# jaeyoungchoilab/Topsicle

Measured on AMD Instinct MI355X. Metric: bases_scanned_per_sec, higher is better.
Workload: dtype u8

## Files before the change

topsicle_amd/csrc/tps_device.h:

```cpp
#pragma once
#include <stdint.h>
#include "../../include/topsicle_hip.h"

#ifdef TPS_EMU
#define TPS_DEV static inline
#define TPS_HD static inline
#define TPS_PHASE for (int tid = 0; tid < tps::NT; ++tid)
#define TPS_SYNC() ((void)0)
#define TPS_UNROLL
#define TPS_NOVEC
#define TPS_PIN_S(x) ((void)0)
#define TPS_PIN_V(x) ((void)0)
#else
#define TPS_DEV __device__ __forceinline__
#define TPS_HD __host__ __device__ inline
__device__ __forceinline__ int tps_fresh_lane() {
    int t = (int)(threadIdx.x & 63u);
    asm volatile("" : "+v"(t));
    return t;
}
#define TPS_PHASE for (int tid = tps_fresh_lane(), once_ = 1; once_; once_ = 0)
#define TPS_SYNC() do { __builtin_amdgcn_fence(__ATOMIC_SEQ_CST, "wavefront"); __builtin_amdgcn_wave_barrier(); } while (0)
#define TPS_UNROLL _Pragma("unroll")
#define TPS_NOVEC _Pragma("clang loop vectorize(disable) interleave(disable) unroll(disable)")
// ... 89 lines not shown
TPS_DEV uint32_t lut_at(const uint32_t* lut, uint32_t v4, uint32_t amask) { return *(const uint32_t*)((const char*)lut + (v4 & amask)); }
#define lut_at_tile lut_at
#else
TPS_DEV uint32_t lut_at(const uint32_t* lut, uint32_t v4, uint32_t amask) {
    typedef const __attribute__((address_space(3))) uint32_t* lptr_t;
    const uint32_t base = (uint32_t)(uintptr_t)(lptr_t)lut;
    return *(lptr_t)(uintptr_t)((v4 & amask) | base);
}
#ifdef TPS_DIAG_NOCONF
TPS_DEV uint32_t lut_at_tile(const uint32_t* lut, uint32_t v4, uint32_t amask) {
    typedef const __attribute__((address_space(3))) uint32_t* lptr_t;
    const uint32_t base = (uint32_t)(uintptr_t)(lptr_t)lut;
    return *(lptr_t)(uintptr_t)((((v4 & amask) >> 30) | ((threadIdx.x & 63u) << 2)) | base);
}
#else
#define lut_at_tile lut_at
#endif
#endif

#ifndef TPS_WIDE16_MODE
#define TPS_WIDE16_MODE 1
#endif
#ifdef TPS_EMU
TPS_DEV uint32_t lut16_at(const uint32_t* lut, uint32_t v2, uint32_t amask1) { return *(const uint16_t*)((const char*)lut + (v2 & amask1)); }
#define lut16_at_wide lut16_at
#else
TPS_DEV uint32_t lut16_at(const uint32_t* lut, uint32_t v2, uint32_t amask1) {
    typedef const __attribute__((address_space(3))) uint16_t* lptr16_t;
    const uint32_t base = (uint32_t)(uintptr_t)(const __attribute__((address_space(3))) uint32_t*)lut;
    return *(lptr16_t)(uintptr_t)((v2 & amask1) | base);
}
TPS_DEV uint32_t lut16_at_wide(const uint32_t* lut, uint32_t v2, uint32_t amask1) {
    uint32_t h = lut16_at(lut, v2, amask1);
#if TPS_WIDE16_MODE == 1
    asm("" : "+v"(h));
#endif
    return h;
}
#endif

#ifdef TPS_EMU
TPS_DEV void g16_store(uint64_t base, uint32_t i, uint32_t v) { ((uint16_t*)(uintptr_t)base)[i] = (uint16_t)v; }
TPS_DEV uint32_t g16_load(uint64_t base, uint32_t i) { return ((const uint16_t*)(uintptr_t)base)[i]; }
#else
TPS_DEV void g16_store(uint64_t base, uint32_t i, uint32_t v) {
    typedef __attribute__((address_space(1))) uint16_t* gp_t;
    ((gp_t)(uintptr_t)base)[i] = (uint16_t)v;
}
TPS_DEV uint32_t g16_load(uint64_t base, uint32_t i) {
    typedef const __attribute__((address_space(1))) uint16_t* gp_t;
    return ((gp_t)(uintptr_t)base)[i];
}
#endif

#ifdef TPS_EMU
TPS_DEV void g32_store(uint64_t base, uint32_t i, uint32_t v) { ((uint32_t*)(uintptr_t)base)[i] = v; }
TPS_DEV uint32_t g32_load(uint64_t base, uint32_t i) { return ((const uint32_t*)(uintptr_t)base)[i]; }
#else
TPS_DEV void g32_store(uint64_t base, uint32_t i, uint32_t v) {
    typedef __attribute__((address_space(1))) uint32_t* gp_t;
    ((gp_t)(uintptr_t)base)[i] = v;
}
TPS_DEV uint32_t g32_load(uint64_t base, uint32_t i) {
    typedef const __attribute__((address_space(1))) uint32_t* gp_t;
    return ((gp_t)(uintptr_t)base)[i];
}
#endif

TPS_DEV uint32_t mulhi32(uint32_t x, uint32_t y) { return (uint32_t)(((uint64_t)x * (uint64_t)y) >> 32); }
#ifdef TPS_EMU
TPS_DEV uint32_t mul24(uint32_t x, uint32_t y) { return (x & 0xFFFFFFu) * (y & 0xFFFFFFu); }
#else
TPS_DEV uint32_t mul24(uint32_t x, uint32_t y) { return (x & 0xFFFFFFu) * (y & 0xFFFFFFu); }
#endif
#ifdef TPS_EMU
TPS_DEV uint32_t add_bytes(uint32_t v, uint32_t acc) { return acc + (v & 255u) + ((v >> 8) & 255u) + ((v >> 16) & 255u) + (v >> 24); }
#else
TPS_DEV uint32_t add_bytes(uint32_t v, uint32_t acc) { return __builtin_amdgcn_sad_u8(v, 0u, acc); }
#endif

constexpr int cgcd(int a, int b) { return b == 0 ? a : cgcd(b, a % b); }
constexpr int clog2(int x) { return x <= 1 ? 0 : 1 + clog2(x / 2); }

#if defined(TPS_EMU) || !defined(TPS_STAMPS)
#define TPS_STAMP(i) ((void)0)
#else
#define TPS_STAMP(i) do { if (a.stamps && (threadIdx.x & 63u) == 0) a.stamps[r * 16 + (i)] = __builtin_readcyclecounter(); } while (0)
#endif
#if defined(TPS_EMU) || !defined(TPS_STAMPS)
#define TPS_PP_STAMP(i) ((void)0)
#else
#define TPS_PP_STAMP(i) do { if (w0 == 0 && a.stamps && (threadIdx.x & 63u) == 0) a.stamps[tc.rd * 16 + (i)] = __builtin_readcyclecounter(); } while (0)
#endif

struct PatInfo {
    int32_t P, k;
    uint32_t kmask;
    uint32_t all_mask;
    uint32_t so_mask;
    uint32_t dup_mask;
    int32_t n_periods;
    int32_t period[8];
    uint32_t period_pat[8];
    uint32_t hash_mul, hash_shift;
};

struct ScanArgs {
    const uint32_t* seq2;
    const uint16_t* inv;
    const tps_read_desc* desc;
    const uint8_t* tails_in;
    const uint32_t* lut;
    const uint32_t* lut_img;
    const uint32_t* pair_img;
    tps_read_result* results;
    int32_t* c_start;
    int32_t* c_end;
    const int64_t* win_off;
    int32_t* sums;
    uint16_t* sums16;
    const int64_t* win_off16;
    uint8_t* raw;
    uint64_t* stamps;
    int32_t raw_m;
    const int64_t* raw_win_off;
    const int32_t* order;
    int64_t n_reads;
    PatInfo pat;
    tps_params prm;
    int32_t variant;
    int32_t lut_n;
    int32_t seq_dw;
    int32_t head_dw;
    int32_t nblk_cap;
    int32_t spans_per_tile;
    int32_t span_dw;
    int32_t blk_log2;
    int32_t rec_rs;
    int32_t tot_dw;
    int32_t blk_dw;
    int32_t lc_cap;
    uint32_t jump_magic;
    int32_t q, r, lw;
    int32_t lc16;
    int32_t lc_global;
    int32_t lc_stride;
    uint16_t* lc_scratch;
    int32_t pair_n;
    int32_t tile_cap;
    int32_t tw;
    uint32_t tw_magic;
    int32_t tile_full;
    int32_t wpg;
    int32_t pp_d;
    int32_t so_fast;
    int32_t val_on;
    int32_t seq_alias;
    int32_t lut_fields;
    int32_t lut16;
    int32_t xt_alias;
    int32_t xt_own;
    int32_t pair16;
};

struct BinsegArgs {
    const int32_t* sums;
    const int64_t* win_off;
    int32_t* bkp;
    double* gain;
    int64_t n_reads;
// ... 774 lines not shown
    uint64_t lc_g;
    uint16_t* sw16;
    int64_t rd;
};
TPS_DEV TileConst tile_const(const ScanArgs& a, int64_t r) {
    TileConst t;
    t.lc_g = a.lc_global ? (uint64_t)(uintptr_t)(a.lc_scratch + r * (int64_t)a.lc_stride) : 0ull;
    t.sw16 = a.sums16 + (a.win_off16 ? a.win_off16[r] : 0);
    t.rd = r;
    t.q = (int32_t)uniform((uint32_t)a.q); t.r = (int32_t)uniform((uint32_t)a.r);
    t.jump = uniform((uint32_t)a.prm.jump); t.jump_magic = uniform(a.jump_magic);
    t.lc_cap = uniform((uint32_t)a.lc_cap); t.lc16 = uniform((uint32_t)a.lc16);
    TPS_PIN_S(t.q); TPS_PIN_S(t.r); TPS_PIN_S(t.jump); TPS_PIN_S(t.jump_magic); TPS_PIN_S(t.lc_cap); TPS_PIN_S(t.lc16);
    return t;
}

#ifndef TPS_RAW_M
#define TPS_RAW_M 1
#endif
template <int S>
struct Geo {
    static constexpr int B = 8;
    static constexpr int LOG2B = 3;
    static constexpr int C = 8;
    static constexpr int LOG2C = 3;
    static constexpr int POS = B * S;
    static constexpr int WDW = (POS + 13 + 15) / 16;
};
constexpr int SEQ_LEAD = 4;
template <int S, bool FULL>
struct TileGeo {
    static constexpr int LANES = FULL ? NT : NT - 1;
    static constexpr int BASES = LANES * Geo<S>::POS + 13 + 15;
    static constexpr int NQ = (63 + BASES + 63) / 64;
    static constexpr int PF = (NQ + NT - 1) / NT;
    static constexpr int SEQ_TILE = SEQ_LEAD + 4 * NQ + 4;
    static constexpr int SEQ = SEQ_TILE < 144 ? 144 : SEQ_TILE;
};
constexpr bool tile_full_default(int s) { return s >= 1; }

template <int S, bool FULL, int XM = 0>
TPS_DEV Lds carve_fused(uint32_t* base, uint32_t* lut, const ScanArgs& a) {
    constexpr bool XTA = XM == 1;
    constexpr int BLK = 9 * NT + (XM == 0 ? 2 : XM == 1 ? 1 : 0) * XLANES, ROW = NT * Geo<S>::B + NT, SEQ = TileGeo<S, FULL>::SEQ;
    const int VAL = a.val_on ? ((SEQ + 4 + 3) / 4) * 2 : 0;
    static_assert(BLK % 4 == 0 && ROW % 4 == 0 && MISC_DW % 4 == 0 && SEQ % 4 == 0, "seq2 must be 16-byte aligned");
    static_assert(BLK + ROW - SEQ >= HIST_DW && BLK + ROW - SEQ >= 4 * NT, "step 1 counts in front of the aliased bases");
    Lds l;
    l.lut2 = lut - a.pair_n;
    l.lut = lut;
    l.lshift = (a.lut16 && !a.lut_fields && !a.pair16) ? LUT_M16 : (a.lut_fields && a.lut16) ? LUT_F16 : a.lut_fields ? LUT_FIELDS : 16;
    l.blk = base;
    l.XPC = base;
    l.XF = base + 9 * NT;
    l.XT = l.XF + XLANES;
    l.G = l.Gp = base; l.C0 = l.C1 = (uint16_t*)base;
    l.row = base + BLK;
    l.misc = l.row + ROW;
    l.Tot = l.misc + MISC_DW;
    uint32_t* p = l.Tot + 4;
    if (a.seq_alias) {
        l.seq2 = base + (BLK + ROW - SEQ);
    } else {
        l.seq2 = p;
        p += SEQ;
    }
    l.val = (uint16_t*)p;
    p += VAL;
    l.Lc = p;
    l.Lc16 = (uint16_t*)p;
    l.Tc = p + ((a.lc16 && a.lc_global) ? 0 : ((a.lc_cap + 3) / 4) * 2);
    if (XTA) l.XT = a.xt_own ? p + lc_dw(a) : l.seq2;
    if (XM == 2) {
        l.XF = p + lc_dw(a);
        l.XT = l.XF + XLANES;
    }
    return l;
}

#ifdef TPS_EMU
inline int& emu_counter(int i) { static int c[8] = {0, 0, 0, 0, 0, 0, 0, 0}; return c[i]; }
#endif
TPS_DEV uint32_t pack_hi_lo(uint32_t hi_src, uint32_t lo_src) { return perm(hi_src, lo_src, 0x07060100u); }

template <int S, bool SO, bool INV, int RPT, bool PAIR, bool RAW>
TPS_DEV void tile_fused_s(const ScanArgs& a, const TileConst& tc, const Lds& l, int delta, int w0, int tile, int nw_tile,
                          int64_t out_base, uint64_t& s_total, int64_t r) {
    constexpr bool RZ = RPT == 0;
    typedef Geo<S> g_;
    constexpr int WDW = g_::WDW, B = g_::B, LOG2B = g_::LOG2B, POS = g_::POS;
    constexpr int RS = NT + NT / B;
    const PatInfo& pat = a.pat;
    const int rp = RPT >= 0 ? RPT : tc.r, q = tc.q;
    const uint32_t amask = pat.kmask << 2;
    TPS_PHASE {
        const int span = tid;
        const int p0 = delta + span * POS;
        const uint32_t sh2 = (uint32_t)((p0 - 1) & 15) * 2u;
        const int d0 = (p0 - 1) >> 4;
        uint32_t w[WDW];
        {
            uint32_t prev = l.seq2[d0];
            TPS_UNROLL
            for (int i = 0; i < WDW; ++i) {
                uint32_t nx = l.seq2[d0 + i + 1];
                w[i] = alignbit(nx, prev, sh2);
                prev = nx;
            }
        }
        uint32_t cnt = 0, run_or = 0;
        uint32_t gs[B], c0s[B];
        uint32_t* xs = l.row + span * (B + 1);
        uint32_t* xpc = l.XPC + span * (B + 1);
        if constexpr (PAIR) {
            static_assert(!SO && !INV, "pair lookups need per-position independence");
            constexpr int NP = S / 2, NH = NP + (S & 1);
            const uint32_t amask2 = (pat.kmask << 4) | 0xCu;
            const int rpe = rp & ~1;
            uint32_t hc[NH], hn[NH];
            auto v4_at = [&](int p) -> uint32_t {
                const int dw = p >> 4, bit = p & 15;
                return bit ? alignbit(dw + 1 < WDW ? w[dw + 1] : 0u, w[dw], 2u * bit) : w[dw];
            };
            auto fetch = [&](int blk, uint32_t* hh) {
                TPS_UNROLL
                for (int j = 0; j < NP; ++j) hh[j] = lut_at(l.lut2, v4_at(blk * S + 2 * j), amask2);
                if (S & 1) hh[NP] = lut_at(l.lut, v4_at(blk * S + S - 1), amask);
            };
            fetch(0, hc);
            TPS_UNROLL
            for (int blk = 0; blk < B; ++blk) {
                if (blk + 1 < B) fetch(blk + 1, hn);
                uint32_t g = 0;
                c0s[blk] = cnt;
                if (RZ) xpc[blk] = pack_hi_lo(run_or, cnt);
                TPS_UNROLL
                for (int j = 0; j < NH; ++j) {
                    if (!RZ) {
                        if (2 * j == rpe) {
                            uint32_t c1 = cnt, pp = run_or | g;
                            if (rp & 1) {
                                const uint32_t h1 = lut_at(l.lut, v4_at(blk * S + 2 * j), amask);
                                c1 += h1;
                                pp |= h1;
                            }
                            xpc[blk] = pack_hi_lo(pp, c1);
                        }
                    }
                    g |= hc[j];
                    cnt += hc[j];
                }
                gs[blk] = g;
                run_or |= g;
                TPS_UNROLL
                for (int j = 0; j < NH; ++j) hc[j] = hn[j];
            }
        } else {
            uint32_t hc[S], hn[S];
            auto fetch = [&](int blk, uint32_t* hh, int cnt_) {
                TPS_UNROLL
                for (int i = 0; i < S; ++i) {
                    if (i < cnt_) {
                        const int p = blk * S + i;
                        const int dw = p >> 4, bit = p & 15;
                        uint32_t v4 = bit ? alignbit(dw + 1 < WDW ? w[dw + 1] : 0u, w[dw], 2u * bit) : w[dw];
                        uint32_t h;
// ... 269 lines not shown
        TPS_PHASE {
            const uint32_t carry = (uint32_t)s_total;
            if (tid == 0) { l.misc[M_INVALID] = 0; l.misc[M_NTIE] = 0; }
            if (tc.lc16 && tid == 0) l.Tc[tile] = carry;
            uint32_t c = c_lo + (uint32_t)tid;
            uint32_t w = c * jump - (uint32_t)w0;
            TPS_NOVEC
            for (int t = 0; t < passes; ++t) {
                if (c < c_hi) {
                    const uint32_t pre = l.row[w + (w >> LOG2B)];
                    if (tc.lc16) {
                        if (tc.lc_g) g16_store(tc.lc_g, c, pre);
                        else l.Lc16[c] = (uint16_t)pre;
                    } else if (tc.lc_g) {
                        g32_store(tc.lc_g, c, carry + pre);
                    } else {
                        l.Lc[c] = carry + pre;
                    }
                }
                c += NT;
                w += NT * jump;
            }
        }
    }
    s_total += gsum;
    TPS_SYNC();
}

TPS_DEV void tile_candidates(const TileConst& tc, const Lds& l, int w0, int tile, int nw_tile, uint64_t& s_total) {
    constexpr int B = 8, LOG2B = 3;
    const uint32_t gsum = wg_exclusive_scan(l.row, NT * B, &l.misc[M_SCAN], LOG2B);
    const uint32_t jump = tc.jump;
    const uint32_t c_lo = div_jump((uint32_t)w0 + jump - 1u, tc.jump_magic);
    uint32_t c_hi = div_jump((uint32_t)(w0 + nw_tile) + jump - 1u, tc.jump_magic);
    if (c_hi > tc.lc_cap) c_hi = tc.lc_cap;
    const int passes = c_hi > c_lo ? (int)((c_hi - c_lo + NT - 1) / NT) : 0;
    TPS_PHASE {
        const uint32_t carry = (uint32_t)s_total;
        if (tid == 0) { l.misc[M_INVALID] = 0; l.misc[M_NTIE] = 0; }
        if (tc.lc16 && tid == 0) l.Tc[tile] = carry;
        uint32_t c = c_lo + (uint32_t)tid;
        uint32_t w = c * jump - (uint32_t)w0;
        TPS_NOVEC
        for (int t = 0; t < passes; ++t) {
            if (c < c_hi) {
                const uint32_t pre = l.row[w + (w >> LOG2B)];
                if (tc.lc16) {
                    if (tc.lc_g) g16_store(tc.lc_g, c, pre);
                    else l.Lc16[c] = (uint16_t)pre;
                } else if (tc.lc_g) {
                    g32_store(tc.lc_g, c, carry + pre);
                } else {
                    l.Lc[c] = carry + pre;
                }
            }
            c += NT;
            w += NT * jump;
        }
    }
    s_total += gsum;
    TPS_SYNC();
}

#ifndef TPS_PP_RPT
#define TPS_PP_RPT 1
#endif
#ifndef TPS_PP_PAIRF
#define TPS_PP_PAIRF 1
#endif
#ifndef TPS_XPAD
#define TPS_XPAD 1
#endif
#ifndef TPS_LC_TILE
#define TPS_LC_TILE 1
#endif
#ifndef TPS_STORE_AUX
#define TPS_STORE_AUX 2
#endif
#ifdef TPS_EMU
TPS_DEV void g_store_sw8(uint16_t* tile_out, int lane, int nw_tile, const uint32_t* v) {
    for (int i = 0; i < 8; ++i)
        if (8 * lane + i < nw_tile) tile_out[8 * lane + i] = (uint16_t)v[i];
}
#else
TPS_DEV void g_store_sw8(uint16_t* tile_out, int lane, int nw_tile, const uint32_t* v) {
    typedef unsigned int v4u __attribute__((ext_vector_type(4)));
    const __amdgpu_buffer_rsrc_t rs = __builtin_amdgcn_make_buffer_rsrc((void*)tile_out, 0, ((nw_tile + 1) & ~1) * 2, 0x00020000);
    v4u t;
    t.x = v[0] | (v[1] << 16); t.y = v[2] | (v[3] << 16); t.z = v[4] | (v[5] << 16); t.w = v[6] | (v[7] << 16);
    __builtin_amdgcn_raw_buffer_store_b128(t, rs, lane * 16, 0, TPS_STORE_AUX);
}
#endif
#ifdef TPS_EMU
TPS_DEV void g_store16_clamped(uint32_t* base, int n_dw, int cdw, const u32x4& t) {
    const uint32_t v[4] = {t.x, t.y, t.z, t.w};
    for (int i = 0; i < 4; ++i)
        if (cdw + i < n_dw) base[cdw + i] = v[i];
}
#else
TPS_DEV void g_store16_clamped(uint32_t* base, int n_dw, int cdw, const u32x4& t) {
    typedef unsigned int v4u __attribute__((ext_vector_type(4)));
    const __amdgpu_buffer_rsrc_t rs = __builtin_amdgcn_make_buffer_rsrc((void*)base, 0, n_dw * 4, 0x00020000);
    v4u x;
    x.x = t.x; x.y = t.y; x.z = t.z; x.w = t.w;
#ifndef TPS_NO_RAW_STORE
    __builtin_amdgcn_raw_buffer_store_b128(x, rs, cdw * 4, 0, TPS_STORE_AUX);
#endif
}
#endif
template <int S, bool INV, int RPT, bool PAIR, bool ROTZ, int CD_ = 0, bool P16_ = false>
TPS_DEV void tile_lc_s(const ScanArgs& a, const TileConst& tc, const Lds& l, int delta, int w0, int tile, int nw_tile,
                       int64_t out_base, uint64_t& s_total, int64_t r) {
    static_assert(!(PAIR && INV), "pair lookups need per-position independence");
    constexpr int CD = CD_;
    static_assert(CD == 0 || (!PAIR && !INV && CD <= S), "chain corrections: single lookups on clean tiles, period <= slide");
    static_assert(!(P16_ && CD_ > 0), "the 16-bit pair table is for tables without self-overlap");
    constexpr bool RZ = RPT == 0;
    constexpr bool M16 = CD > 0 || P16_;
    constexpr int LS = M16 ? 1 : 2;
    constexpr bool XPAD = TPS_XPAD != 0;
    typedef Geo<S> g_;
    auto xf_at = [&](int lane_) -> uint32_t& { return XPAD ? l.XPC[lane_ * (g_::B + 1) + g_::B] : l.XF[lane_]; };
    auto xt_at = [&](int lane_) -> uint32_t& { return XPAD ? l.row[lane_ * (g_::B + 1) + g_::B] : l.XT[lane_]; };
    constexpr int B = g_::B, LOG2B = g_::LOG2B, POS = g_::POS;
    constexpr int LB = CD;
    constexpr int WDW = (LB + POS + 13 + 15) / 16;
    static_assert(CD > 0 || WDW == g_::WDW, "the plain tiles keep Geo's register footprint");
    const PatInfo& pat = a.pat;
    int rp = RPT >= 0 ? RPT : tc.r, q = tc.q;
    TPS_PIN_S(q);
    if (RPT < 0) TPS_PIN_S(rp);
    const uint32_t amask = pat.kmask << LS;
    uint32_t sfx[B], c0s[B], xf_own = 0;
#ifdef TPS_EMU
    uint32_t sfx_keep[NT][B], c0_keep[NT][B], xf_keep[NT];
#endif
    uint32_t lane_chain = 0;
    uint32_t pair_lo = 0, pair_hi = 0;
#ifdef TPS_EMU
    uint32_t pair_keep[NT][2];
#endif
    auto chain_len = [&](int tp, uint32_t pm) -> int {
        constexpr int CD = CD_ > 0 ? CD_ : 1;
        auto occ = [&](int pos) -> bool { return uniform(lut_mask(l.lut, l.lshift, pat, v_at(l.seq2, delta + pos)) & pm) != 0u; };
        const int tend = NT * POS;
        int c = 3;
        while (tp + c * CD < tend && occ(tp + c * CD)) ++c;
        return c;
    };
    auto chain_windows = [&](int tp, int c, int ln) {
        constexpr int CD = CD_ > 0 ? CD_ : 1;
        const int lw = a.lw;
        auto w_in = [&](int e) -> int { const int x = e - lw + 1; return x <= 0 ? 0 : (x + S - 1) / S; };
        auto cur_of = [&](int w) -> int {
            const int a0 = w * S - tp, a1 = w * S + lw - 1 - tp;
            int jlo = a0 <= 0 ? 0 : (a0 + CD - 1) / CD, jhi = a1 < 0 ? -1 : a1 / CD;
            if (jhi > c - 1) jhi = c - 1;
            return jhi > jlo ? (jhi - jlo) >> 1 : 0;
        };
        const int wf = w_in(tp < 0 ? 0 : tp);
        int wb = (tp + (c - 1) * CD) / S + 1;
        if (wb > NT * B - 1) wb = NT * B - 1;
        for (int w = wf + ln; w <= wb; w += NT) {
            const int cur = cur_of(w), prev = w == wf ? 0 : cur_of(w - 1);
            if (cur != prev) lds_add(&l.row[w + (w >> LOG2B)], (uint32_t)(cur - prev));
        }
    };
    TPS_PHASE {
        const int span = tid;
        const int p0 = delta + span * POS;
        const int bo = 2 * (p0 - LB) - LS;
        const uint32_t sh2 = (uint32_t)(bo & 31);
        const int d0 = bo >> 5;
        uint32_t w[WDW];
        {
            uint32_t prev = l.seq2[d0];
            TPS_UNROLL
            for (int i = 0; i < WDW; ++i) {
                uint32_t nx = l.seq2[d0 + i + 1];
                w[i] = alignbit(nx, prev, sh2);
                prev = nx;
            }
        }
        auto v4_at = [&](int p) -> uint32_t {
            const int dw = (p + LB) >> 4, bit = (p + LB) & 15;
            return bit ? alignbit(dw + 1 < WDW ? w[dw + 1] : 0u, w[dw], 2u * bit) : w[dw];
        };
        uint32_t cnt = 0, run_or = 0;
        uint32_t gs[B];
        pair_lo = pair_hi = 0;
        uint32_t* xpc = l.XPC + span * (B + 1);
        if constexpr (PAIR) {
            constexpr int NP = S / 2, NH = NP + (S & 1);
            const uint32_t amask2 = M16 ? ((pat.kmask << 3) | 0x6u) : ((pat.kmask << 4) | 0xCu);
            const int rpe = rp & ~1;
            uint32_t hc[NH], hn[NH];
            auto fetch = [&](int blk, uint32_t* hh) {
                TPS_UNROLL
                for (int j = 0; j < NP; ++j) hh[j] = M16 ? lut16_at(l.lut2, v4_at(blk * S + 2 * j), amask2) : lut_at_tile(l.lut2, v4_at(blk * S + 2 * j), amask2);
                if (S & 1) hh[NP] = M16 ? lut16_at(l.lut, v4_at(blk * S + S - 1), amask) : lut_at_tile(l.lut, v4_at(blk * S + S - 1), amask);
            };
            fetch(0, hc);
            TPS_UNROLL
            for (int blk = 0; blk < B; ++blk) {
                if (blk + 1 < B) fetch(blk + 1, hn);
                uint32_t g = 0;
                c0s[blk] = cnt;
                if (RZ) xpc[blk] = M16 ? ((run_or << 16) | cnt) : pack_hi_lo(run_or, cnt);
                TPS_UNROLL
                for (int j = 0; j < NH; ++j) {
                    if (!RZ) {
                        if (2 * j == rpe) {
                            uint32_t c1 = cnt, pp = run_or | g;
                            if (rp & 1) {
                                const uint32_t h1 = M16 ? lut16_at(l.lut, v4_at(blk * S + 2 * j), amask) : lut_at(l.lut, v4_at(blk * S + 2 * j), amask);
                                c1 = M16 ? c1 + (uint32_t)popc(h1) : c1 + h1;
                                pp |= h1;
                            }
                            xpc[blk] = M16 ? ((pp << 16) | c1) : pack_hi_lo(pp, c1);
                        }
                    }
                    g |= hc[j];
                    cnt = M16 ? cnt + (uint32_t)popc(hc[j]) : cnt + hc[j];
                }
                gs[blk] = g;
                run_or |= g;
                TPS_UNROLL
                for (int j = 0; j < NH; ++j) hc[j] = hn[j];
            }
        } else {
            uint32_t hc[S], hn[S];
            auto fetch = [&](int blk, uint32_t* hh, int cnt_) {
                TPS_UNROLL
                for (int i = 0; i < S; ++i) {
                    if (i < cnt_) {
                        const int p = blk * S + i;
                        uint32_t h = M16 ? lut16_at_wide(l.lut, v4_at(p), amask) : lut_at(l.lut, v4_at(p), amask);
                        if (INV) {
                            if (h && invalid_at(l.val, p0 + p, pat.k)) h = 0;
                        }
                        hh[i] = h;
                    } else {
                        hh[i] = 0;
                    }
                }
            };
            fetch(0, hc, S);
            constexpr int NB_ = CD > 0 ? CD : 1;
            uint32_t hb[NB_];
            if constexpr (CD > 0) {
// ... 102 lines not shown
                    return (uint32_t)(popc(pair_lo) + popc(pair_hi & ((1u << (n - 32)) - 1u)));
                };
                if ((pair_lo | pair_hi) != 0u) {
                    uint32_t* xpc = l.XPC + lane * (B + 1);
                    TPS_UNROLL
                    for (int blk = 0; blk < B; ++blk) {
                        const uint32_t pe = below(blk * S + (RZ ? 0 : RPT));
                        if (pe) lds_add(&xpc[blk], pe << PS);
                        c0s[blk] += below(blk * S + CD) << PS;
                    }
                    const uint32_t pt = below(64) << PS;
                    xf_own += pt;
                    lds_add(&xf_at(lane), pt);
                }
                uint32_t prev_hi, next_lo;
#ifdef TPS_EMU
                prev_hi = lane > 0 ? pair_keep[lane - 1][1] : 0u;
                const uint32_t prev_lo_ = lane > 0 ? pair_keep[lane - 1][0] : 0u;
                next_lo = lane + 1 < NT ? pair_keep[lane + 1][0] : 0u;
#else
                prev_hi = (uint32_t)__builtin_amdgcn_ds_bpermute(((lane + NT - 1) & (NT - 1)) << 2, (int)pair_hi);
                const uint32_t prev_lo_ = (uint32_t)__builtin_amdgcn_ds_bpermute(((lane + NT - 1) & (NT - 1)) << 2, (int)pair_lo);
                next_lo = (uint32_t)__builtin_amdgcn_ds_bpermute(((lane + 1) & (NT - 1)) << 2, (int)pair_lo);
                if (lane == 0) prev_hi = 0u;
                if (lane == NT - 1) next_lo = 0u;
#endif
                const uint64_t pm64 = ((uint64_t)pair_hi << 32) | pair_lo;
                const uint64_t pv64 = lane > 0 ? (((uint64_t)prev_hi << 32) | prev_lo_) : 0ull;
                const uint64_t before = (pm64 << CD) | (pv64 >> (POS - CD));
                const uint64_t after = (pm64 >> CD) | ((uint64_t)(next_lo & ((1u << CD) - 1u)) << (POS - CD));
                const uint64_t lim = POS >= 64 ? ~0ull : ((1ull << POS) - 1ull);
                const uint64_t h3 = pm64 & ~before & after & lim;
                head3_lo = (uint32_t)h3; head3_hi = (uint32_t)(h3 >> 32);
#ifdef TPS_EMU
                for (int j = 0; j < B; ++j) c0_keep[tid][j] = c0s[j];
                xf_keep[tid] = xf_own;
                head3_keep[tid][0] = head3_lo; head3_keep[tid][1] = head3_hi;
#endif
            }
#ifdef TPS_EMU
            bool tile_long = false;
            for (int t = 0; t < NT; ++t) tile_long = tile_long || (head3_keep[t][0] | head3_keep[t][1]) != 0u;
#else
            const bool tile_long = __builtin_amdgcn_ballot_w64((head3_lo | head3_hi) != 0u) != 0;
#endif
            if (tile_long) {
                TPS_PHASE {
                    TPS_UNROLL
                    for (int i = 0; i < B + 1; ++i) l.row[tid + i * NT] = 0;
                }
                TPS_SYNC();
                auto one_owner = [&](int src, uint32_t h_lo, uint32_t h_hi, auto&& each_lane) {
                    while (h_lo | h_hi) {
                        int e;
                        if (h_lo) { e = ffs0(h_lo); h_lo &= h_lo - 1u; }
                        else { e = 32 + ffs0(h_hi); h_hi &= h_hi - 1u; }
                        const int te = src * POS + e;
                        const uint32_t pm = uniform(lut_mask(l.lut, l.lshift, pat, v_at(l.seq2, delta + te)));
                        const int c = chain_len(te - CD, pm);
                        each_lane(te - CD, c);
                    }
                };
#ifdef TPS_EMU
                for (int src = 0; src < NT; ++src)
                    one_owner(src, head3_keep[src][0], head3_keep[src][1], [&](int tp, int c) { for (int ln = 0; ln < NT; ++ln) chain_windows(tp, c, ln); });
#else
                {
                    const int ln = tps_fresh_lane();
                    uint64_t owners = __builtin_amdgcn_ballot_w64((head3_lo | head3_hi) != 0u);
                    while (owners) {
                        const int src = __builtin_ctzll(owners);
                        owners &= owners - 1ull;
                        const uint32_t h_lo = (uint32_t)__builtin_amdgcn_readlane((int)head3_lo, src), h_hi = (uint32_t)__builtin_amdgcn_readlane((int)head3_hi, src);
                        one_owner(src, h_lo, h_hi, [&](int tp, int c) { chain_windows(tp, c, ln); });
                    }
                }
#endif
                lane_chain = 1u;
            }
        }
    }
    TPS_SYNC();
    if (w0 == 0) TPS_STAMP(6);
    const int rot = ROTZ ? 0 : (q & (B - 1)), dl0 = q >> LOG2B;
    const int brk = B - rot;
    uint32_t sw[B], ltot = 0;
#ifdef TPS_EMU
    uint32_t sw_keep[NT][B], tot_keep[NT];
#endif
    TPS_PHASE {
#ifdef TPS_EMU
        for (int j = 0; j < B; ++j) { sfx[j] = sfx_keep[tid][j]; c0s[j] = c0_keep[tid][j]; }
        xf_own = xf_keep[tid];
#endif
        const int lane = tid;
        const uint32_t* pe = l.XPC + (lane + dl0) * (B + 1) + rot;
        uint32_t ev[B];
        TPS_UNROLL
        for (int j = 0; j < B; ++j) ev[j] = pe[j + ((!ROTZ && j >= brk) ? 1 : 0)];
        uint32_t orw = 0, sumw = xf_own;
        TPS_NOVEC
        for (int t = 1; t < dl0; ++t) {
            const uint32_t v = xf_at(lane + t);
            orw |= v;
            sumw += v;
        }
        uint32_t orb = orw, sumb = sumw;
        if (!ROTZ) {
            const uint32_t vb = xf_at(lane + dl0);
            orb |= vb;
            sumb += vb;
        }
        const uint32_t am = pat.all_mask << 16;
        uint32_t run = 0;
        TPS_UNROLL
        for (int j = 0; j < B; ++j) {
            const bool far_ = !ROTZ && j >= brk;
            const uint32_t e = ev[j], fo = far_ ? orb : orw, fs = far_ ? sumb : sumw;
            const uint32_t m = sfx[j] | e | fo;
            const uint32_t c = (e - c0s[j] + fs) & 0xFFFFu;
            sw[j] = (CD > 0 ? (c & 0xFFu) - (c >> 8) : c) + (uint32_t)popc(~m & am);
            run += sw[j];
        }
        ltot = run;
#ifdef TPS_EMU
        for (int j = 0; j < B; ++j) sw_keep[tid][j] = sw[j];
        tot_keep[tid] = ltot;
#endif
    }
    if constexpr (CD > 0) {
#ifdef TPS_EMU
        const bool tile_chain = lane_chain != 0;
        if (tile_chain) {
            ++emu_counter(5);
            uint32_t acc = 0;
            for (int t = 0; t < NT; ++t) {
                uint32_t tot = 0;
                for (int j = 0; j < B; ++j) { acc += l.row[t * (B + 1) + j]; sw_keep[t][j] += acc; tot += sw_keep[t][j]; }
                tot_keep[t] = tot;
            }
        } else {
            ++emu_counter(6);
        }
#else
        const bool tile_chain = lane_chain != 0;
        if (tile_chain) {
            uint32_t pd[B], dt = 0;
            TPS_PHASE {
                const uint32_t* pr = l.row + tid * (B + 1);
                TPS_UNROLL
                for (int j = 0; j < B; ++j) { dt += pr[j]; pd[j] = dt; }
            }
            uint32_t inc = dt;
            inc += (uint32_t)__builtin_amdgcn_update_dpp(0, (int)inc, 0x111, 0xf, 0xf, false);
            inc += (uint32_t)__builtin_amdgcn_update_dpp(0, (int)inc, 0x112, 0xf, 0xf, false);
            inc += (uint32_t)__builtin_amdgcn_update_dpp(0, (int)inc, 0x114, 0xf, 0xf, false);
            inc += (uint32_t)__builtin_amdgcn_update_dpp(0, (int)inc, 0x118, 0xf, 0xf, false);
            inc += (uint32_t)__builtin_amdgcn_update_dpp(0, (int)inc, 0x142, 0xa, 0xf, false);
            inc += (uint32_t)__builtin_amdgcn_update_dpp(0, (int)inc, 0x143, 0xc, 0xf, false);
            const uint32_t dbase = inc - dt;
            uint32_t run = 0;
            TPS_UNROLL
            for (int j = 0; j < B; ++j) { sw[j] += dbase + pd[j]; run += sw[j]; }
            ltot = run;
        }
#endif
    }
    uint32_t lexc = 0;
#ifdef TPS_EMU
    uint32_t exc_keep[NT];
    { uint32_t acc = 0; for (int t = 0; t < NT; ++t) { exc_keep[t] = acc; acc += tot_keep[t]; } }
#else
    {
        uint32_t inc = ltot;
        inc += (uint32_t)__builtin_amdgcn_update_dpp(0, (int)inc, 0x111, 0xf, 0xf, false);
        inc += (uint32_t)__builtin_amdgcn_update_dpp(0, (int)inc, 0x112, 0xf, 0xf, false);
        inc += (uint32_t)__builtin_amdgcn_update_dpp(0, (int)inc, 0x114, 0xf, 0xf, false);
        inc += (uint32_t)__builtin_amdgcn_update_dpp(0, (int)inc, 0x118, 0xf, 0xf, false);
        inc += (uint32_t)__builtin_amdgcn_update_dpp(0, (int)inc, 0x142, 0xa, 0xf, false);
        inc += (uint32_t)__builtin_amdgcn_update_dpp(0, (int)inc, 0x143, 0xc, 0xf, false);
        lexc = inc - ltot;
    }
#endif
    TPS_PHASE {
#ifdef TPS_EMU
        for (int j = 0; j < B; ++j) sw[j] = sw_keep[tid][j];
        lexc = exc_keep[tid];
#endif
        const int lane = tid;
#ifndef TPS_NO_SW_STORE
        g_store_sw8(tc.sw16 + w0, lane, nw_tile, sw);
#endif
        uint32_t* pr = l.row + lane * (B + 1);
        uint32_t run = 0;
        TPS_UNROLL
        for (int j = 0; j < B; ++j) { pr[j] = run; run += sw[j]; }
        xt_at(lane) = lexc;
    }
    TPS_SYNC();
    if (w0 == 0) TPS_STAMP(12);
    const uint32_t gsum = uniform(l.row[nw_tile + (nw_tile >> LOG2B)] + xt_at(nw_tile >> LOG2B));
    {
        const uint32_t jump = tc.jump;
        const uint32_t c_lo = div_jump((uint32_t)w0 + jump - 1u, tc.jump_magic);
        uint32_t c_hi = div_jump((uint32_t)(w0 + nw_tile) + jump - 1u, tc.jump_magic);
        if (c_hi > tc.lc_cap) c_hi = tc.lc_cap;
        const int passes = c_hi > c_lo ? (int)((c_hi - c_lo + NT - 1) / NT) : 0;
        TPS_PHASE {
            const uint32_t carry = (uint32_t)s_total;
            if (tid == 0) { l.misc[M_INVALID] = 0; l.misc[M_NTIE] = 0; }
            if (tc.lc16 && tid == 0) l.Tc[tile] = carry;
            uint32_t c = c_lo + (uint32_t)tid;
            uint32_t w = c * jump - (uint32_t)w0;
            TPS_NOVEC
            for (int t = 0; t < passes; ++t) {
                if (c < c_hi) {
                    const uint32_t pre = l.row[w + (w >> LOG2B)] + xt_at((int)(w >> LOG2B));
                    if (tc.lc16) {
                        if (tc.lc_g) g16_store(tc.lc_g, c, pre);
                        else l.Lc16[c] = (uint16_t)pre;
                    } else if (tc.lc_g) {
                        g32_store(tc.lc_g, c, carry + pre);
                    } else {
                        l.Lc[c] = carry + pre;
                    }
                }
                c += NT;
                w += NT * jump;
            }
        }
    }
    s_total += gsum;
    TPS_SYNC();
    (void)r;
}

template <int S>
struct GeoPP {
    static constexpr int B = 8, POS = B * S, LBK = 16;
    static constexpr int WDW = (1 + LBK + POS + 6 + 7 + 15) / 16;
};
constexpr uint32_t PP_BIAS = 14;
TPS_DEV void pp_expand(uint32_t ne, uint32_t no, uint32_t* b) {
    b[0] = ne & 0x0F0F0F0Fu;
    b[1] = (ne >> 4) & 0x0F0F0F0Fu;
    b[2] = no & 0x0F0F0F0Fu;
    b[3] = (no >> 4) & 0x0F0F0F0Fu;
}

template <int S, int D, int CD = 0, bool F16 = false, int RPT = -1, bool PAIRF = false>
TPS_DEV bool tile_pp_s(const ScanArgs& a, const TileConst& tc, const Lds& l, int delta, int w0, int tile, int nw_tile,
                       int64_t out_base, uint64_t& s_total) {
    static_assert(CD == 0 || (D == 0 && CD <= 6), "chain detection runs on the tile without self-overlap logic");
    static_assert(RPT < S, "r is a position inside a block");
    static_assert(!PAIRF || (D == 0 && CD == 0 && !F16 && RPT >= 0 && (RPT & 1) == 0), "pair lookups: plain tiles, the partial block ends between two pairs");
    constexpr int B = 8, POS = B * S, LBK = D > 0 ? 2 * D + 2 : 0;
    constexpr int WDW = (1 + LBK + POS + 6 + 7 + 15) / 16;
    constexpr int DH = D > 0 ? D : 1;
    constexpr int AHEAD = (D > 0 && 2 * D > S) ? 2 * D - S : 0;
    constexpr uint32_t M3 = 0x33333333u;
    const PatInfo& pat = a.pat;
    int rp = RPT >= 0 ? RPT : tc.r, q = tc.q;
    if constexpr (RPT < 0) TPS_PIN_S(rp);
    TPS_PIN_S(q);
    constexpr int LS = F16 ? 1 : 2;
    const uint32_t amask = pat.kmask << LS;
    uint32_t* ende = l.XPC;
    uint32_t* endo = l.row;
    uint32_t* tne = ende + B;
    uint32_t* tno = endo + B;
    uint32_t* carry = l.misc + M_SCAN;
    const int cblk = a.tw & (B - 1), clane = a.tw >> 3;
    uint32_t cold[7];
    TPS_UNROLL
    for (int i = 0; i < 7; ++i) cold[i] = (D > 0) ? uniform(carry[i]) : 0u;
    auto picked_before_tile = [&](int pos, int fidx) -> bool {
        uint32_t cv = 0;
        TPS_UNROLL
        for (int i = 0; i < DH; ++i) cv = (pos - (delta - DH) == i) ? cold[i] : cv;
        return w0 != 0 && ((cv >> (2 * fidx)) & 1u) != 0;
    };
#ifdef TPS_EMU
    uint32_t keep[NT][2 * B + 3];
    if (CD == 0) ++emu_counter(0);
#endif
    uint32_t ve[B], vo[B], chm = 0, chw = 0, unc = 0;
    uint32_t chain_any = 0;
    TPS_PHASE {
        const int span = tid;
        const int p0 = delta + span * POS;
        const int bo = 2 * (p0 - LBK) - LS;
        const uint32_t sh2 = (uint32_t)(bo & 31);
        const int d0 = bo >> 5;
        uint32_t w[WDW];
        {
            uint32_t prev = l.seq2[d0];
            TPS_UNROLL
            for (int i = 0; i < WDW; ++i) {
                uint32_t nx = l.seq2[d0 + i + 1];
                w[i] = alignbit(nx, prev, sh2);
                prev = nx;
            }
        }
        auto look = [&](int p) -> uint32_t {
            const int idx = p + LBK, dw = idx >> 4, bit = idx & 15;
            const uint32_t v4 = bit ? alignbit(dw + 1 < WDW ? w[dw + 1] : 0u, w[dw], 2u * bit) : w[dw];
            if constexpr (F16) {
                const uint32_t m = lut16_at(l.lut, v4, amask);
                return mul24(m, m);
            }
            const uint32_t h = lut_at(l.lut, v4, amask);
            return h;
        };
        uint32_t pk[LBK + POS + AHEAD + 1];
        uint32_t tv[POS + 1];
// ... 1381 lines not shown
```

Measured before the change: 3579 billion.

## Pack window sums as u16 pairs and emit candidate prefixes per lane

In the ROTZ, non-CD path, per-window sums are now computed two at a time with packed 16-bit add and subtract, and the packed words are stored directly. This removes the shift/or repacking in the sw store. When each lane covers at most two candidates (jump >= 4, 32-bit global Lc), lanes write candidate prefix sums straight from their registers, so the separate LDS-reading candidate pass is skipped. The all_mask masking is folded into orw/orb up front. ISA marker asm comments are added behind a build flag.

```diff
diff --git a/topsicle_amd/csrc/tps_device.h b/topsicle_amd/csrc/tps_device.h
--- a/topsicle_amd/csrc/tps_device.h
+++ b/topsicle_amd/csrc/tps_device.h
@@ -195,10 +195,15 @@
 constexpr int cgcd(int a, int b) { return b == 0 ? a : cgcd(b, a % b); }
 constexpr int clog2(int x) { return x <= 1 ? 0 : 1 + clog2(x / 2); }
 
-#if defined(TPS_EMU) || !defined(TPS_STAMPS)
+#if defined(TPS_ISA_MARKS) && !defined(TPS_EMU)
+#define TPS_STAMP(i) asm volatile(";tps_stamp %0" ::"i"(i))
+#define TPS_ISA_MARK(id) asm volatile(";tps_mark %0" ::"i"(id))
+#elif defined(TPS_EMU) || !defined(TPS_STAMPS)
 #define TPS_STAMP(i) ((void)0)
+#define TPS_ISA_MARK(id) ((void)(id))
 #else
 #define TPS_STAMP(i) do { if (a.stamps && (threadIdx.x & 63u) == 0) a.stamps[r * 16 + (i)] = __builtin_readcyclecounter(); } while (0)
+#define TPS_ISA_MARK(id) ((void)(id))
 #endif
 #if defined(TPS_EMU) || !defined(TPS_STAMPS)
 #define TPS_PP_STAMP(i) ((void)0)
@@ -1139,6 +1144,15 @@
 inline int& emu_counter(int i) { static int c[8] = {0, 0, 0, 0, 0, 0, 0, 0}; return c[i]; }
 #endif
 TPS_DEV uint32_t pack_hi_lo(uint32_t hi_src, uint32_t lo_src) { return perm(hi_src, lo_src, 0x07060100u); }
+#ifdef TPS_EMU
+TPS_DEV uint32_t pk_u16_sub(uint32_t a, uint32_t b) { return ((a - b) & 0xFFFFu) | (((a >> 16) - (b >> 16)) << 16); }
+TPS_DEV uint32_t pk_u16_add(uint32_t a, uint32_t b) { return ((a + b) & 0xFFFFu) | (((a >> 16) + b) << 16); }
+#else
+typedef unsigned short tps_u16x2 __attribute__((ext_vector_type(2)));
+TPS_DEV tps_u16x2 as_u16x2(uint32_t v) { return __builtin_bit_cast(tps_u16x2, v); }
+TPS_DEV uint32_t pk_u16_sub(uint32_t a, uint32_t b) { return __builtin_bit_cast(uint32_t, as_u16x2(a) - as_u16x2(b)); }
+TPS_DEV uint32_t pk_u16_add(uint32_t a, uint32_t b) { return __builtin_bit_cast(uint32_t, as_u16x2(a) + (tps_u16x2)((unsigned short)b)); }
+#endif
 
 template <int S, bool SO, bool INV, int RPT, bool PAIR, bool RAW>
 TPS_DEV void tile_fused_s(const ScanArgs& a, const TileConst& tc, const Lds& l, int delta, int w0, int tile, int nw_tile,
@@ -1574,12 +1588,23 @@
     for (int i = 0; i < 8; ++i)
         if (8 * lane + i < nw_tile) tile_out[8 * lane + i] = (uint16_t)v[i];
 }
+TPS_DEV void g_store_sw8p(uint16_t* tile_out, int lane, int nw_tile, const uint32_t* p) {
+    for (int i = 0; i < 8; ++i)
+        if (8 * lane + i < nw_tile) tile_out[8 * lane + i] = (uint16_t)(p[i >> 1] >> (16 * (i & 1)));
+}
 #else
 TPS_DEV void g_store_sw8(uint16_t* tile_out, int lane, int nw_tile, const uint32_t* v) {
     typedef unsigned int v4u __attribute__((ext_vector_type(4)));
     const __amdgpu_buffer_rsrc_t rs = __builtin_amdgcn_make_buffer_rsrc((void*)tile_out, 0, ((nw_tile + 1) & ~1) * 2, 0x00020000);
     v4u t;
     t.x = v[0] | (v[1] << 16); t.y = v[2] | (v[3] << 16); t.z = v[4] | (v[5] << 16); t.w = v[6] | (v[7] << 16);
+    __builtin_amdgcn_raw_buffer_store_b128(t, rs, lane * 16, 0, TPS_STORE_AUX);
+}
+TPS_DEV void g_store_sw8p(uint16_t* tile_out, int lane, int nw_tile, const uint32_t* p) {
+    typedef unsigned int v4u __attribute__((ext_vector_type(4)));
+    const __amdgpu_buffer_rsrc_t rs = __builtin_amdgcn_make_buffer_rsrc((void*)tile_out, 0, ((nw_tile + 1) & ~1) * 2, 0x00020000);
+    v4u t;
+    t.x = p[0]; t.y = p[1]; t.z = p[2]; t.w = p[3];
     __builtin_amdgcn_raw_buffer_store_b128(t, rs, lane * 16, 0, TPS_STORE_AUX);
 }
 #endif
@@ -1658,6 +1683,8 @@
             if (cur != prev) lds_add(&l.row[w + (w >> LOG2B)], (uint32_t)(cur - prev));
         }
     };
+    constexpr int MK = 10 * S + 1000 * (RPT + 1) + 100000 * ROTZ + 1000000 * PAIR + 10000000 * INV + 100000000 * (CD > 0 || P16_);
+    TPS_ISA_MARK(MK + 1);
     TPS_PHASE {
         const int span = tid;
         const int p0 = delta + span * POS;
@@ -1926,11 +1953,13 @@
     }
     TPS_SYNC();
     if (w0 == 0) TPS_STAMP(6);
+    TPS_ISA_MARK(MK + 2);
     const int rot = ROTZ ? 0 : (q & (B - 1)), dl0 = q >> LOG2B;
     const int brk = B - rot;
-    uint32_t sw[B], ltot = 0;
-#ifdef TPS_EMU
-    uint32_t sw_keep[NT][B], tot_keep[NT];
+    constexpr bool SWP = CD == 0 && !M16 && ROTZ;
+    uint32_t sw[B], swp[B / 2], ltot = 0;
+#ifdef TPS_EMU
+    uint32_t sw_keep[NT][B], swp_keep[NT][B / 2], tot_keep[NT];
 #endif
     TPS_PHASE {
 #ifdef TPS_EMU
@@ -1956,22 +1985,43 @@
             sumb += vb;
         }
         const uint32_t am = pat.all_mask << 16;
+        orw |= ~am;
+        orb |= ~am;
         uint32_t run = 0;
+        if constexpr (SWP) {
+#ifdef TPS_EMU
+            if (tid == 0) ++emu_counter(3);
+#endif
+            uint32_t lo_lo = 0x05040100u;
+            TPS_PIN_S(lo_lo);
+            TPS_UNROLL
+            for (int j = 0; j < B; j += 2) {
+                const uint32_t ep = perm(ev[j + 1], ev[j], lo_lo), cp = perm(c0s[j + 1], c0s[j], lo_lo);
+                const uint32_t d = pk_u16_add(pk_u16_sub(ep, cp), sumw);
+                const uint32_t p = (uint32_t)popc(~(sfx[j] | ev[j] | orw)) + d;
+                swp[j >> 1] = p + ((uint32_t)popc(~(sfx[j + 1] | ev[j + 1] | orw)) << 16);
+                sw[j] = swp[j >> 1] & 0xFFFFu;
+                sw[j + 1] = swp[j >> 1] >> 16;
+                run += sw[j] + sw[j + 1];
+            }
+        } else {
         TPS_UNROLL
         for (int j = 0; j < B; ++j) {
             const bool far_ = !ROTZ && j >= brk;
             const uint32_t e = ev[j], fo = far_ ? orb : orw, fs = far_ ? sumb : sumw;
-            const uint32_t m = sfx[j] | e | fo;
             const uint32_t c = (e - c0s[j] + fs) & 0xFFFFu;
-            sw[j] = (CD > 0 ? (c & 0xFFu) - (c >> 8) : c) + (uint32_t)popc(~m & am);
+            sw[j] = (CD > 0 ? (c & 0xFFu) - (c >> 8) : c) + (uint32_t)popc(~(sfx[j] | e | fo));
             run += sw[j];
         }
+        }
         ltot = run;
 #ifdef TPS_EMU
         for (int j = 0; j < B; ++j) sw_keep[tid][j] = sw[j];
+        if (SWP) for (int j = 0; j < B / 2; ++j) swp_keep[tid][j] = swp[j];
         tot_keep[tid] = ltot;
 #endif
     }
+    TPS_ISA_MARK(MK + 3);
     if constexpr (CD > 0) {
 #ifdef TPS_EMU
         const bool tile_chain = lane_chain != 0;
@@ -2026,30 +2076,48 @@
         lexc = inc - ltot;
     }
 #endif
+    bool lane_cands = false;
+    if constexpr (CD == 0 && !M16) lane_cands = tc.lc_g != 0ull && !tc.lc16 && tc.jump >= 4u;
     TPS_PHASE {
 #ifdef TPS_EMU
         for (int j = 0; j < B; ++j) sw[j] = sw_keep[tid][j];
+        if (SWP) for (int j = 0; j < B / 2; ++j) swp[j] = swp_keep[tid][j];
         lexc = exc_keep[tid];
 #endif
         const int lane = tid;
 #ifndef TPS_NO_SW_STORE
-        g_store_sw8(tc.sw16 + w0, lane, nw_tile, sw);
+        if constexpr (SWP) g_store_sw8p(tc.sw16 + w0, lane, nw_tile, swp);
+        else g_store_sw8(tc.sw16 + w0, lane, nw_tile, sw);
 #endif
         uint32_t* pr = l.row + lane * (B + 1);
         uint32_t run = 0;
         TPS_UNROLL
         for (int j = 0; j < B; ++j) { pr[j] = run; run += sw[j]; }
         xt_at(lane) = lexc;
+        if (lane_cands) {
+#ifdef TPS_EMU
+            if (tid == 0) ++emu_counter(7);
+#endif
+            const uint32_t carry = (uint32_t)s_total + lexc;
+            const uint32_t wl = (uint32_t)(lane * B), wa = (uint32_t)w0 + wl;
+            const uint32_t c = mulhi32(wa + tc.jump - 1u, tc.jump_magic);
+            const uint32_t f = c * tc.jump - wa;
+            if (f < (uint32_t)B && wl + f < (uint32_t)nw_tile && c < tc.lc_cap) g32_store(tc.lc_g, c, carry + pr[f]);
+            const uint32_t f2 = f + tc.jump;
+            if (f2 < (uint32_t)B && wl + f2 < (uint32_t)nw_tile && c + 1u < tc.lc_cap) g32_store(tc.lc_g, c + 1u, carry + pr[f2]);
+        }
     }
     TPS_SYNC();
     if (w0 == 0) TPS_STAMP(12);
+    TPS_ISA_MARK(MK + 4);
     const uint32_t gsum = uniform(l.row[nw_tile + (nw_tile >> LOG2B)] + xt_at(nw_tile >> LOG2B));
     {
         const uint32_t jump = tc.jump;
         const uint32_t c_lo = div_jump((uint32_t)w0 + jump - 1u, tc.jump_magic);
         uint32_t c_hi = div_jump((uint32_t)(w0 + nw_tile) + jump - 1u, tc.jump_magic);
         if (c_hi > tc.lc_cap) c_hi = tc.lc_cap;
-        const int passes = c_hi > c_lo ? (int)((c_hi - c_lo + NT - 1) / NT) : 0;
+        const int passes = (c_hi > c_lo && !lane_cands) ? (int)((c_hi - c_lo + NT - 1) / NT) : 0;
+        TPS_ISA_MARK(MK + 6);
         TPS_PHASE {
             const uint32_t carry = (uint32_t)s_total;
             if (tid == 0) { l.misc[M_INVALID] = 0; l.misc[M_NTIE] = 0; }
@@ -2075,6 +2143,7 @@
         }
     }
     s_total += gsum;
+    TPS_ISA_MARK(MK + 5);
     TPS_SYNC();
     (void)r;
 }
```

Result: faster. 3702 billion (median of 6 runs) (+3.5%).
